# ychalier/transflow

Hardware: AMD Instinct MI355X
Metric: frames/sec (Farneback+remap) (higher is better)
Workload: dtype f32; 1 GPU; 4k: one clip of T=256 3840x2160 uint8 frames sharded over the ranks (rank r owns pairs shard_range(255, r, 1) + a one-frame halo), Farneback pyr_scale=0.5 levels=5 winsize=15 iterations=3 poly_n=5 poly_sigma=1.2 flags=0, BACKWARD post_process, moveref layer (reset random p=0.5 through a float mask, u drawn on the GPU), 1 RGB pixmap source, render; clip_frames=256, equal_batches=False

## Files before the change

transflow_amd/csrc/common.h:

```cpp
#pragma once
#include <hip/hip_runtime.h>

#include <cstdarg>
#include <cstdint>
#include <cstdio>
#include <cstdlib>
#include <string>
#include <vector>

#include "../../include/tfhip.h"

#define TF_API extern "C" __attribute__((visibility("default")))

namespace tf {

int set_error(int code, const char *fmt, ...) __attribute__((format(printf, 2, 3)));
hipStream_t stream();
hipStream_t main_stream();
int side_stream(int which, hipStream_t *out);
int ensure_init();

enum Opt { OPT_FB_FUSED = 0, OPT_FB_FUSE_MIN_PX, OPT_FB_NO_SHARE, OPT_FB_NO_OVERLAP, OPT_REMAP_PX, OPT_REMAP_NO_PACK, OPT_REMAP_KEEP_RGBA,
           OPT_PROF_LEVELS, OPT_FB_EXACT_SUMS, OPT_FB_CHAIN, OPT_FB_SEGS, OPT_REMAP_QUAD, OPT_JD_PAR_SUB_BYTES,
           OPT_JD_PAR_GROUP_SUBS, OPT_JD_PAR_STAGED, OPT_REMAP_LEAN, OPT_COUNT };
long option(Opt which);

#ifdef TF_EXPERIMENT
inline long tune(const char *env, long dflt)
{
    const char *v = getenv(env);
    return v ? atol(v) : dflt;
}
inline const char *tune_str(const char *env) { return getenv(env); }
#else
constexpr long tune(const char *, long dflt) { return dflt; }
constexpr const char *tune_str(const char *) { return nullptr; }
#endif

struct StreamScope {
    explicit StreamScope(hipStream_t s);
    ~StreamScope();
    hipStream_t prev;
};

#define TF_HIP(expr)                                                                              \
    do {                                                                                          \
        hipError_t _e = (expr);                                                                   \
        if (_e != hipSuccess)                                                                     \
            return tf::set_error(TF_ERR_HIP, "%s failed: %s (%s:%d)", #expr, hipGetErrorString(_e), \
                                 __FILE__, __LINE__);                                             \
    } while (0)

#define TF_TRY(expr)        \
    do {                    \
        int _rc = (expr);   \
        if (_rc != TF_OK)   \
            return _rc;     \
    } while (0)

#define TF_REQUIRE(cond, ...)                         \
    do {                                              \
        if (!(cond))                                  \
            return tf::set_error(TF_ERR_ARG, __VA_ARGS__); \
    } while (0)

struct ProfScope {
    explicit ProfScope(const char *name);
    ~ProfScope();
    const char *name;
    hipEvent_t a, b;
};
bool prof_enabled();

template <typename K, typename... Args>
inline int launch(const char *name, K kernel, dim3 grid, dim3 block, size_t smem, Args... args)
{
    if (grid.x == 0 || grid.y == 0 || grid.z == 0)
        return TF_OK;
    {
        ProfScope ps(name);
        hipLaunchKernelGGL(kernel, grid, block, smem, stream(), args...);
    }
    hipError_t e = hipGetLastError();
    if (e != hipSuccess)
        return set_error(TF_ERR_HIP, "launch %s failed: %s", name, hipGetErrorString(e));
    return TF_OK;
}

struct DevBuf {
    void *p = nullptr;
    size_t bytes = 0;
    bool borrowed = false;
    DevBuf() = default;
    DevBuf(const DevBuf &) = delete;
    DevBuf &operator=(const DevBuf &) = delete;
    ~DevBuf() { release(); }
    int alloc(size_t n);
    void borrow(void *ptr, size_t n);
    void release();
    template <typename T> T *as() const { return reinterpret_cast<T *>(p); }
};

struct PinnedBuf {
    void *p = nullptr;
    PinnedBuf() = default;
    PinnedBuf(const PinnedBuf &) = delete;
    PinnedBuf &operator=(const PinnedBuf &) = delete;
    ~PinnedBuf() { release(); }
    int alloc(size_t n);
    void release();
    template <typename T> T *as() const { return reinterpret_cast<T *>(p); }
};

struct Event {
    hipEvent_t e = nullptr;
    Event() = default;
    Event(const Event &) = delete;
    Event &operator=(const Event &) = delete;
    ~Event() { release(); }
    int create();
    void release();
    operator hipEvent_t() const { return e; }
};

inline unsigned cdiv(size_t a, size_t b) { return (unsigned)((a + b - 1) / b); }

struct FastDiv {
    uint32_t m;
    int s1, s2;
};
inline FastDiv fast_div_setup(uint32_t d)
{
    int s = 0;
    while ((1ull << s) < d)
        s++;
    FastDiv f;
    f.m = (uint32_t)(((1ull << 32) * ((1ull << s) - d)) / d + 1);
    f.s1 = s < 1 ? s : 1;
    f.s2 = s > 1 ? s - 1 : 0;
    return f;
}
__device__ __forceinline__ uint32_t fast_div(uint32_t t, FastDiv f)
{
    const uint32_t hi = __umulhi(t, f.m);
    return (((t - hi) >> f.s1) + hi) >> f.s2;
}

__device__ __forceinline__ float clip_nan(float v, float lo, float hi) { return v != v ? v : fminf(fmaxf(v, lo), hi); }

__device__ __forceinline__ int clampi(int v, int lo, int hi) { return v < lo ? lo : (v > hi ? hi : v); }

struct PpLabels {
    const char *clip, *fwd_scatter, *fwd_resolve, *ops;
};
constexpr PpLabels PP_FB{"pp_clip", "pp_fwd_scatter", "pp_fwd_resolve", "pp_ops"};
constexpr PpLabels PP_FLOW{"flow_pp_clip", "flow_pp_fwd_scatter", "flow_pp_fwd_resolve", "flow_pp_ops"};
int pp_ops(float2 *flow, int W, int H, int n_ops, const tf_flow_op *ops, const float *mask_dev, const PpLabels &lb);
int pp_scatter(const float2 *flow, int W, int H, int *winner, const PpLabels &lb);
int pp_direction(void *flow, bool wide, int W, int H, int direction, int *winner, const PpLabels &lb);

}
```

transflow_amd/csrc/fb_pyramid.hip:

```cpp
#include "fb_common.h"

namespace {

#ifndef TF_PX_TH
#define TF_PX_TH 16
#endif
constexpr int PX_TW = 64, PX_TH = TF_PX_TH;

__global__ void k_polyexp(const float *__restrict__ img, float *__restrict__ R, int Wk, int Hk, PolyConst pc)
{
    extern __shared__ float s_mem[];
    const int n = pc.n;
    const int LW = PX_TW + 2 * n;
    const int LH = PX_TH + 2 * n;
    float *sI = s_mem;
    float *sT = s_mem + LH * LW;
    const int pi = blockIdx.z;
    const size_t Nk = (size_t)Wk * Hk;
    const float *src = img + (size_t)pi * Nk;
    const int x0 = blockIdx.x * PX_TW, y0 = blockIdx.y * PX_TH;
    for (int idx = threadIdx.x; idx < LH * LW; idx += blockDim.x) {
        int ry = idx / LW, cx = idx % LW;
        int y = clampi(y0 - n + ry, 0, Hk - 1), x = clampi(x0 - n + cx, 0, Wk - 1);
        sI[idx] = src[(size_t)y * Wk + x];
    }
    __syncthreads();
    for (int idx = threadIdx.x; idx < PX_TH * LW; idx += blockDim.x) {
        int ty = idx / LW, cx = idx % LW;
        int y = y0 + ty;
        const float c = sI[(ty + n) * LW + cx];
        float t0 = c * pc.g[0], t1 = 0.f, t2 = 0.f;
        for (int k = 1; k <= n; k++) {
            int ya = max(y - k, 0), yb = min(y + k, Hk - 1);
            float a = sI[(ya - y0 + n) * LW + cx];
            float b = sI[(yb - y0 + n) * LW + cx];
            float p = a + b;
            t0 = t0 + pc.g[k] * p;
            t1 = t1 + pc.xg[k] * (b - a);
            t2 = t2 + pc.xxg[k] * p;
        }
        if (y >= Hk) {
            t0 = t1 = t2 = 0.f;
        }
        sT[(0 * PX_TH + ty) * LW + cx] = t0;
        sT[(1 * PX_TH + ty) * LW + cx] = t1;
        sT[(2 * PX_TH + ty) * LW + cx] = t2;
    }
    __syncthreads();
    float *dst = R + (size_t)pi * 5 * Nk;
    for (int idx = threadIdx.x; idx < PX_TH * PX_TW; idx += blockDim.x) {
        int ty = idx / PX_TW, cx = idx % PX_TW;
        int x = x0 + cx, y = y0 + ty;
        if (x >= Wk || y >= Hk)
            continue;
        const float *T0 = sT + (0 * PX_TH + ty) * LW + cx + n;
        const float *T1 = sT + (1 * PX_TH + ty) * LW + cx + n;
        const float *T2 = sT + (2 * PX_TH + ty) * LW + cx + n;
        float g0 = pc.g[0];
        double b1 = T0[0] * g0, b2 = 0, b3 = T1[0] * g0, b4 = 0, b5 = T2[0] * g0, b6 = 0;
        for (int k = 1; k <= n; k++) {
            double tg = T0[k] + T0[-k];
            g0 = pc.g[k];
            b1 = __builtin_fma(tg, (double)g0, b1);
            b4 = __builtin_fma(tg, (double)pc.xxg[k], b4);
            b2 += (T0[k] - T0[-k]) * pc.xg[k];
            b3 += (T1[k] + T1[-k]) * g0;
            b6 += (T1[k] - T1[-k]) * pc.xg[k];
            b5 += (T2[k] + T2[-k]) * g0;
        }
        size_t o = (size_t)y * Wk + x;
        const float v[5] = {(float)(b3 * pc.ig11), (float)(b2 * pc.ig11), (float)(b1 * pc.ig03 + b5 * pc.ig33),
                            (float)(b1 * pc.ig03 + b4 * pc.ig33), (float)(b6 * pc.ig55)};
        r_store_px(dst, Nk, o, v);
    }
}

typedef float float2w __attribute__((ext_vector_type(2), aligned(4)));

template <int N>
__device__ __forceinline__ void polyexp_vertical4(const f32x2 (&v)[4 + 2 * N], const PolyConst &pc, float *T0, float *T1,
                                                  float *T2, int LW)
{
#pragma unroll
    for (int q = 0; q < 4; q++) {
        const f32x2 c = v[q + N];
        f32x2 t0 = c * pc.g[0], t1 = {0.f, 0.f}, t2 = {0.f, 0.f};
#pragma unroll
        for (int k = 1; k <= N; k++) {
            const f32x2 a = v[q + N - k], b = v[q + N + k];
            const f32x2 p = a + b;
            t0 = t0 + pc.g[k] * p;
            t1 = t1 + pc.xg[k] * (b - a);
            t2 = t2 + pc.xxg[k] * p;
        }
        *reinterpret_cast<f32x2 *>(T0 + q * LW) = t0;
        *reinterpret_cast<f32x2 *>(T1 + q * LW) = t1;
        *reinterpret_cast<f32x2 *>(T2 + q * LW) = t2;
    }
}

template <int N>
__global__ void __launch_bounds__(256)
k_polyexp_t(const float *__restrict__ img, float *__restrict__ R, int Wk, int Hk, PolyConst pc)
{
    constexpr int TW = PX_TW, TH = PX_TH, LW = TW + 2 * N, LH = TH + 2 * N;
    __shared__ float sI[LH * LW];
    __shared__ float sT[3][TH][LW];
    const int pi = blockIdx.z;
    const size_t Nk = (size_t)Wk * Hk;
    const float *src = img + (size_t)pi * Nk;
    const int x0 = blockIdx.x * TW, y0 = blockIdx.y * TH;
    for (int idx = threadIdx.x; idx < LH * LW; idx += 256) {
        int ry = idx / LW, cx = idx - ry * LW;
        int y = clampi(y0 - N + ry, 0, Hk - 1), x = clampi(x0 - N + cx, 0, Wk - 1);
        sI[idx] = src[(size_t)y * Wk + x];
    }
    __syncthreads();
    static_assert(LW % 2 == 0, "column pairs");
    for (int idx = threadIdx.x; idx < (TH / 4) * (LW / 2); idx += 256) {
        const int g = idx / (LW / 2), cx = 2 * (idx - g * (LW / 2));
        f32x2 v[4 + 2 * N];
#pragma unroll
        for (int j = 0; j < 4 + 2 * N; j++)
            v[j] = *reinterpret_cast<const f32x2 *>(&sI[(4 * g + j) * LW + cx]);
        polyexp_vertical4<N>(v, pc, &sT[0][4 * g][cx], &sT[1][4 * g][cx], &sT[2][4 * g][cx], LW);
    }
    __syncthreads();
    float *dst = R + (size_t)pi * 5 * Nk;
    for (int idx = threadIdx.x; idx < TH * (TW / 2); idx += 256) {
        const int ty = idx / (TW / 2), cp = idx - ty * (TW / 2);
        const int x = x0 + 2 * cp, y = y0 + ty;
        if (x >= Wk || y >= Hk)
            continue;
        float w0[2 + 2 * N], w1[2 + 2 * N], w2[2 + 2 * N];
#pragma unroll
        for (int j = 0; j < 2 + 2 * N; j++) {
            w0[j] = sT[0][ty][2 * cp + j];
            w1[j] = sT[1][ty][2 * cp + j];
            w2[j] = sT[2][ty][2 * cp + j];
        }
        float out[2][5];
#pragma unroll
        for (int q = 0; q < 2; q++) {
            const float *T0 = w0 + q + N, *T1 = w1 + q + N, *T2 = w2 + q + N;
            float g0 = pc.g[0];
            double b1 = T0[0] * g0, b2 = 0, b3 = T1[0] * g0, b4 = 0, b5 = T2[0] * g0, b6 = 0;
#pragma unroll
            for (int k = 1; k <= N; k++) {
                double tg = T0[k] + T0[-k];
                g0 = pc.g[k];
                b1 = __builtin_fma(tg, (double)g0, b1);
                b4 = __builtin_fma(tg, (double)pc.xxg[k], b4);
                b2 += (T0[k] - T0[-k]) * pc.xg[k];
                b3 += (T1[k] + T1[-k]) * g0;
                b6 += (T1[k] - T1[-k]) * pc.xg[k];
                b5 += (T2[k] + T2[-k]) * g0;
            }
            out[q][0] = (float)(b3 * pc.ig11);
            out[q][1] = (float)(b2 * pc.ig11);
            out[q][2] = (float)(b1 * pc.ig03 + b5 * pc.ig33);
            out[q][3] = (float)(b1 * pc.ig03 + b4 * pc.ig33);
            out[q][4] = (float)(b6 * pc.ig55);
        }
        const size_t o = (size_t)y * Wk + x;
        if (x + 1 < Wk)
            r_store_px2(dst, Nk, o, out[0], out[1]);
        else
            r_store_px(dst, Nk, o, out[0]);
    }
}

template <int N, int TW, int TH>
__device__ __forceinline__ void tile_expansion(const float *sI, float (*sT)[TH][TW + 2 * N], int x0, int y0, int xr0,
                                               int yr0, int W, int H, const PolyConst &pc, float *dst, size_t Nk)
{
    constexpr int LW = TW + 2 * N;
    const bool interior = x0 - N >= 0 && x0 + TW - 1 + N <= W - 1 && y0 - N >= 0 && y0 + TH - 1 + N <= H - 1;
    for (int idx = threadIdx.x; idx < (TH / 4) * (LW / 2); idx += 256) {
        const int g = idx / (LW / 2), cx = 2 * (idx - g * (LW / 2));
        f32x2 v[4 + 2 * N];
        if (interior) {
#pragma unroll
            for (int j = 0; j < 4 + 2 * N; j++)
                v[j] = *reinterpret_cast<const f32x2 *>(&sI[(4 * g + j) * LW + cx]);
        } else {
            const int xa = clampi(x0 - N + cx, 0, W - 1) - xr0, xb = clampi(x0 - N + cx + 1, 0, W - 1) - xr0;
#pragma unroll
            for (int j = 0; j < 4 + 2 * N; j++) {
                const float *row = sI + (clampi(y0 - N + 4 * g + j, 0, H - 1) - yr0) * LW;
                v[j] = f32x2{row[xa], row[xb]};
            }
        }
        polyexp_vertical4<N>(v, pc, &sT[0][4 * g][cx], &sT[1][4 * g][cx], &sT[2][4 * g][cx], LW);
    }
    __syncthreads();
    for (int idx = threadIdx.x; idx < TH * (TW / 2); idx += 256) {
        const int ty = idx / (TW / 2), cp = idx - ty * (TW / 2);
        const int x = x0 + 2 * cp, y = y0 + ty;
        if (x >= W || y >= H)
            continue;
        float w0[2 + 2 * N], w1[2 + 2 * N], w2[2 + 2 * N];
#pragma unroll
        for (int j = 0; j < 2 + 2 * N; j++) {
            w0[j] = sT[0][ty][2 * cp + j];
            w1[j] = sT[1][ty][2 * cp + j];
            w2[j] = sT[2][ty][2 * cp + j];
        }
        float out[2][5];
#pragma unroll
        for (int q = 0; q < 2; q++) {
            const float *T0 = w0 + q + N, *T1 = w1 + q + N, *T2 = w2 + q + N;
            float g0 = pc.g[0];
            double b1 = T0[0] * g0, b2 = 0, b3 = T1[0] * g0, b4 = 0, b5 = T2[0] * g0, b6 = 0;
#pragma unroll
            for (int k = 1; k <= N; k++) {
                double tg = T0[k] + T0[-k];
                g0 = pc.g[k];
                b1 = __builtin_fma(tg, (double)g0, b1);
                b4 = __builtin_fma(tg, (double)pc.xxg[k], b4);
                b2 += (T0[k] - T0[-k]) * pc.xg[k];
                b3 += (T1[k] + T1[-k]) * g0;
                b6 += (T1[k] - T1[-k]) * pc.xg[k];
                b5 += (T2[k] + T2[-k]) * g0;
            }
            out[q][0] = (float)(b3 * pc.ig11);
            out[q][1] = (float)(b2 * pc.ig11);
            out[q][2] = (float)(b1 * pc.ig03 + b5 * pc.ig33);
            out[q][3] = (float)(b1 * pc.ig03 + b4 * pc.ig33);
            out[q][4] = (float)(b6 * pc.ig55);
        }
        const size_t o = (size_t)y * W + x;
        if (x + 1 < W)
            r_store_px2(dst, Nk, o, out[0], out[1]);
        else
            r_store_px(dst, Nk, o, out[0]);
    }
}

#ifndef TF_EXP_TH0
#define TF_EXP_TH0 16
#endif
#ifndef TF_EXP_TH1
#define TF_EXP_TH1 24
#endif
template <int N>
__global__ void __launch_bounds__(256)
k_level0_polyexp_t(const uint8_t *__restrict__ frames, const int2 *__restrict__ pairs, float *__restrict__ R, int W,
                   int H, float kc, float k1, PolyConst pc)
{
    constexpr int TW = 64, TH = TF_EXP_TH0, LW = TW + 2 * N, LH = TH + 2 * N;
    constexpr int SW = ((LW + 2 + 3 + 3) + 3) & ~3, SH = LH + 2;
    constexpr int RS = (LW + 3) & ~3;
    static_assert(SW >= RS + 4 + 4 && (SH * SW) % 16 == 0, "a group's three dwords stay inside its staged row; sRow 16-byte aligned");
    constexpr int BYTES_A = SH * SW + SH * RS * 4, BYTES_T = 3 * TH * LW * 4;
    constexpr int BYTES_U = ((BYTES_A > BYTES_T ? BYTES_A : BYTES_T) + 15) & ~15;
    __shared__ __attribute__((aligned(16))) uint8_t s_u[BYTES_U];
    __shared__ float sI[LH * LW];
    uint8_t *sS = s_u;
    float *sRow = reinterpret_cast<float *>(s_u + SH * SW);
    float(*sT)[TH][LW] = reinterpret_cast<float(*)[TH][LW]>(s_u);
    const int pi = blockIdx.z;
    const int2 pr = pairs[pi >> 1];
    const uint8_t *src = frames + (size_t)((pi & 1) ? pr.y : pr.x) * W * H;
    const size_t Nk = (size_t)W * H;
    const int x0 = blockIdx.x * TW, y0 = blockIdx.y * TH;
    const int lane = threadIdx.x & 63, wave = threadIdx.x >> 6;
    const int xr0 = max(x0 - N, 0), xr1 = min(x0 + TW - 1 + N, W - 1);
    const int yr0 = max(y0 - N, 0), yr1 = min(y0 + TH - 1 + N, H - 1);
    const int ny = yr1 - yr0 + 1;
    const int xs = (xr0 - 1) & ~3, off = xr0 - 1 - xs;
    const int ncols = xr1 + 1 - xs + 1;
    const bool dwords = (W & 3) == 0 && xs >= 0 && xs + ((ncols + 3) & ~3) <= W;
    constexpr int U = 8;
    if (dwords) {
        const int nq = (ncols + 3) >> 2;
        for (int c = lane; c < nq; c += 64) {
            for (int j0 = wave; j0 < ny + 2; j0 += 4 * U) {
                uint32_t v[U];
#pragma unroll
                for (int u = 0; u < U; u++) {
                    int ry = j0 + 4 * u;
                    if (ry < ny + 2)
                        v[u] = *reinterpret_cast<const uint32_t *>(src + (size_t)reflect101_near(yr0 - 1 + ry, H) * W + xs + 4 * c);
                }
#pragma unroll
                for (int u = 0; u < U; u++) {
                    int ry = j0 + 4 * u;
                    if (ry < ny + 2)
                        *reinterpret_cast<uint32_t *>(sS + ry * SW + 4 * c) = v[u];
                }
            }
        }
    } else {
        for (int c = lane; c < ncols; c += 64) {
            const int x = reflect101_near(xs + c, W);
            for (int j0 = wave; j0 < ny + 2; j0 += 4 * U) {
                uint8_t v[U];
#pragma unroll
                for (int u = 0; u < U; u++) {
                    int ry = j0 + 4 * u;
                    if (ry < ny + 2)
                        v[u] = src[(size_t)reflect101_near(yr0 - 1 + ry, H) * W + x];
                }
#pragma unroll
                for (int u = 0; u < U; u++) {
                    int ry = j0 + 4 * u;
                    if (ry < ny + 2)
                        sS[ry * SW + c] = v[u];
                }
            }
        }
    }
    __syncthreads();
    for (int idx = threadIdx.x; idx < (ny + 2) * (RS / 4); idx += 256) {
        const int ry = idx / (RS / 4), cx = 4 * (idx - ry * (RS / 4));
        const uint32_t *q = reinterpret_cast<const uint32_t *>(sS + ry * SW + cx);
        const uint32_t d0 = q[0], d1 = q[1], d2 = q[2];
        const uint32_t lo = __builtin_amdgcn_alignbyte(d1, d0, off), hi = __builtin_amdgcn_alignbyte(d2, d1, off);
        const float b0 = (float)(lo & 0xff), b1 = (float)((lo >> 8) & 0xff), b2 = (float)((lo >> 16) & 0xff),
                    b3 = (float)(lo >> 24), b4 = (float)(hi & 0xff), b5 = (float)((hi >> 8) & 0xff);
        float *o = sRow + ry * RS + cx;
        *reinterpret_cast<f32x2 *>(o) = f32x2{b1 * kc + (b0 + b2) * k1, b2 * kc + (b1 + b3) * k1};
        *reinterpret_cast<f32x2 *>(o + 2) = f32x2{b3 * kc + (b2 + b4) * k1, b4 * kc + (b3 + b5) * k1};
    }
    __syncthreads();
    for (int idx = threadIdx.x; idx < ny * (RS / 4); idx += 256) {
        const int ry = idx / (RS / 4), cx = 4 * (idx - ry * (RS / 4));
        const float *c = sRow + (ry + 1) * RS + cx;
        const f32x4 m = *reinterpret_cast<const f32x4 *>(c), dn = *reinterpret_cast<const f32x4 *>(c + RS),
                    up = *reinterpret_cast<const f32x4 *>(c - RS);
        f32x4 v = kc * m;
        v += k1 * (dn + up);
        float *o = sI + ry * LW + cx;
        *reinterpret_cast<f32x2 *>(o) = f32x2{v.x, v.y};
        if (cx + 2 < LW)
            *reinterpret_cast<f32x2 *>(o + 2) = f32x2{v.z, v.w};
    }
    __syncthreads();
    tile_expansion<N, TW, TH>(sI, sT, x0, y0, xr0, yr0, W, H, pc, R + (size_t)pi * 5 * Nk, Nk);
}

template <int N>
__global__ void __launch_bounds__(256)
k_level1_polyexp_t(const uint8_t *__restrict__ frames, const int2 *__restrict__ pairs, float *__restrict__ R, int W,
                   int H, float kc, float k1, PolyConst pc)
{
    constexpr int TW = 64, TH = TF_EXP_TH1, LW = TW + 2 * N, LH = TH + 2 * N;
    constexpr int SW = ((2 * LW + 2 + 3 + 3) + 3) & ~3, SH = 2 * LH + 2;
    constexpr int BYTES_A = SH * SW, BYTES_T = 3 * TH * LW * 4;
    constexpr int BYTES_U = ((BYTES_A > BYTES_T ? BYTES_A : BYTES_T) + 15) & ~15;
    __shared__ __attribute__((aligned(16))) uint8_t s_u[BYTES_U];
    __shared__ float sI[LH * LW];
    uint8_t *sS = s_u;
    float(*sT)[TH][LW] = reinterpret_cast<float(*)[TH][LW]>(s_u);
    const int Wk = W >> 1, Hk = H >> 1;
    const int pi = blockIdx.z;
    const int2 pr = pairs[pi >> 1];
    const uint8_t *src = frames + (size_t)((pi & 1) ? pr.y : pr.x) * W * H;
    const size_t Nk = (size_t)Wk * Hk;
    const int x0 = blockIdx.x * TW, y0 = blockIdx.y * TH;
    const int lane = threadIdx.x & 63, wave = threadIdx.x >> 6;
    const int xr0 = max(x0 - N, 0), xr1 = min(x0 + TW - 1 + N, Wk - 1);
    const int yr0 = max(y0 - N, 0), yr1 = min(y0 + TH - 1 + N, Hk - 1);
    const int ny = yr1 - yr0 + 1;
    const int cfirst = 2 * xr0 - 1, rfirst = 2 * yr0 - 1, nrows = 2 * ny + 2;
    const int xs = cfirst >= 0 ? (cfirst & ~3) : cfirst, off = cfirst - xs;
    const int ncols = 2 * xr1 + 2 - xs + 1;
    const bool dwords = (W & 3) == 0 && xs >= 0 && (xs & 3) == 0 && xs + ((ncols + 3) & ~3) <= W;
    constexpr int U = 8;
    if (dwords) {
        const int nq = (ncols + 3) >> 2;
        for (int c = lane; c < nq; c += 64) {
            for (int j0 = wave; j0 < nrows; j0 += 4 * U) {
                uint32_t v[U];
#pragma unroll
                for (int u = 0; u < U; u++) {
                    int ry = j0 + 4 * u;
                    if (ry < nrows)
                        v[u] = *reinterpret_cast<const uint32_t *>(src + (size_t)reflect101_near(rfirst + ry, H) * W + xs + 4 * c);
                }
#pragma unroll
                for (int u = 0; u < U; u++) {
                    int ry = j0 + 4 * u;
                    if (ry < nrows)
                        *reinterpret_cast<uint32_t *>(sS + ry * SW + 4 * c) = v[u];
                }
            }
        }
    } else {
        for (int c = lane; c < ncols; c += 64) {
            const int x = reflect101_near(xs + c, W);
            for (int j0 = wave; j0 < nrows; j0 += 4 * U) {
                uint8_t v[U];
#pragma unroll
                for (int u = 0; u < U; u++) {
                    int ry = j0 + 4 * u;
                    if (ry < nrows)
                        v[u] = src[(size_t)reflect101_near(rfirst + ry, H) * W + x];
                }
#pragma unroll
                for (int u = 0; u < U; u++) {
                    int ry = j0 + 4 * u;
                    if (ry < nrows)
                        sS[ry * SW + c] = v[u];
                }
            }
        }
    }
    __syncthreads();
    static_assert(LW % 2 == 0 && SW >= 2 * LW + 8, "2 x 2 blocks; a block's three dwords stay inside its staged row");
    for (int idx = threadIdx.x; idx < ((ny + 1) >> 1) * (LW / 2); idx += 256) {
        const int by2 = idx / (LW / 2), ry = 2 * by2, cx = 2 * (idx - by2 * (LW / 2));
        float rp[6][4];
#pragma unroll
        for (int dy = 0; dy < 6; dy++) {
            const uint32_t *q = reinterpret_cast<const uint32_t *>(sS + (2 * ry + dy) * SW + 2 * cx);
            const uint32_t d0 = q[0], d1 = q[1], d2 = q[2];
            const uint32_t lo = __builtin_amdgcn_alignbyte(d1, d0, off), hi = __builtin_amdgcn_alignbyte(d2, d1, off);
            const float b0 = (float)(lo & 0xff), b1 = (float)((lo >> 8) & 0xff), b2 = (float)((lo >> 16) & 0xff),
                        b3 = (float)(lo >> 24), b4 = (float)(hi & 0xff), b5 = (float)((hi >> 8) & 0xff);
            rp[dy][0] = b1 * kc + (b0 + b2) * k1;
            rp[dy][1] = b2 * kc + (b1 + b3) * k1;
            rp[dy][2] = b3 * kc + (b2 + b4) * k1;
            rp[dy][3] = b4 * kc + (b3 + b5) * k1;
        }
#pragma unroll
        for (int a = 0; a < 2; a++) {
            float out[2];
#pragma unroll
            for (int b = 0; b < 2; b++) {
                float v00 = kc * rp[2 * a + 1][2 * b], v01 = kc * rp[2 * a + 1][2 * b + 1];
                float v10 = kc * rp[2 * a + 2][2 * b], v11 = kc * rp[2 * a + 2][2 * b + 1];
                v00 += k1 * (rp[2 * a + 2][2 * b] + rp[2 * a][2 * b]);
                v01 += k1 * (rp[2 * a + 2][2 * b + 1] + rp[2 * a][2 * b + 1]);
                v10 += k1 * (rp[2 * a + 3][2 * b] + rp[2 * a + 1][2 * b]);
                v11 += k1 * (rp[2 * a + 3][2 * b + 1] + rp[2 * a + 1][2 * b + 1]);
                const float h0 = v00 * (1.f - 0.5f) + v01 * 0.5f, h1 = v10 * (1.f - 0.5f) + v11 * 0.5f;
                out[b] = h0 * (1.f - 0.5f) + h1 * 0.5f;
            }
            if (ry + a < ny)
                *reinterpret_cast<f32x2 *>(sI + (ry + a) * LW + cx) = f32x2{out[0], out[1]};
        }
    }
    __syncthreads();
    tile_expansion<N, TW, TH>(sI, sT, x0, y0, xr0, yr0, Wk, Hk, pc, R + (size_t)pi * 5 * Nk, Nk);
}

}

namespace tf {
namespace fb {

int fb_polyexp(tf_fb *fb, int w, int h, const ImageRun &run, int k)
{
    const int n = fb->pc.n;
    dim3 grid(cdiv(w, PX_TW), cdiv(h, PX_TH), run.n);
    if (n == 5)
        return launch(lvl_name("fb_polyexp", k), k_polyexp_t<5>, grid, dim3(256), 0, (const float *)fb->imgk(k),
                      fb->Rk(k, run), w, h, fb->pc);
    if (n == 7)
        return launch(lvl_name("fb_polyexp", k), k_polyexp_t<7>, grid, dim3(256), 0, (const float *)fb->imgk(k),
                      fb->Rk(k, run), w, h, fb->pc);
    size_t smem = ((size_t)(PX_TH + 2 * n) * (PX_TW + 2 * n) + 3 * (size_t)PX_TH * (PX_TW + 2 * n)) * sizeof(float);
    return launch(lvl_name("fb_polyexp_generic", k), k_polyexp, grid, dim3(256), smem,
                  (const float *)fb->imgk(k), fb->Rk(k, run), w, h, fb->pc);
}

static bool fb_can_fuse_level(tf_fb *fb, int k)
{
    static const bool off = tune("TF_FB_NO_A1A2", 0) != 0;
    const Level &L = *fb->lv[k];
    return !off && L.W == fb->W && L.H == fb->H && L.ksz == 3 && (fb->pc.n == 5 || fb->pc.n == 7);
}

static bool fb_can_fuse_half_level(tf_fb *fb, int k)
{
    static const bool off = tune("TF_FB_NO_A1A2", 0) != 0;
    const Level &L = *fb->lv[k];
    return !off && 2 * L.W == fb->W && 2 * L.H == fb->H && L.ksz == 3 && (fb->pc.n == 5 || fb->pc.n == 7);
}

static int fb_level1_polyexp(tf_fb *fb, int k, const ImageRun &run)
{
    Level &L = *fb->lv[k];
    dim3 grid(cdiv(L.W, 64), cdiv(L.H, TF_EXP_TH1), run.n);
    const float kc = L.kern_host[1], k1 = L.kern_host[2];
    if (fb->pc.n == 5)
        return launch(lvl_name("fb_level_polyexp", k), k_level1_polyexp_t<5>, grid, dim3(256), 0,
                      (const uint8_t *)fb->frames.as<uint8_t>(), fb->image_list(run), fb->Rk(k, run), fb->W,
                      fb->H, kc, k1, fb->pc);
    return launch(lvl_name("fb_level_polyexp", k), k_level1_polyexp_t<7>, grid, dim3(256), 0,
                  (const uint8_t *)fb->frames.as<uint8_t>(), fb->image_list(run), fb->Rk(k, run), fb->W, fb->H,
                  kc, k1, fb->pc);
}

static int fb_level0_polyexp(tf_fb *fb, int k, const ImageRun &run)
{
    Level &L = *fb->lv[k];
    dim3 grid(cdiv(L.W, 64), cdiv(L.H, TF_EXP_TH0), run.n);
    const float kc = L.kern_host[1], k1 = L.kern_host[2];
    if (fb->pc.n == 5)
        return launch(lvl_name("fb_level_polyexp", k), k_level0_polyexp_t<5>, grid, dim3(256), 0,
                      (const uint8_t *)fb->frames.as<uint8_t>(), fb->image_list(run), fb->Rk(k, run),
                      L.W, L.H, kc, k1, fb->pc);
    return launch(lvl_name("fb_level_polyexp", k), k_level0_polyexp_t<7>, grid, dim3(256), 0,
                  (const uint8_t *)fb->frames.as<uint8_t>(), fb->image_list(run), fb->Rk(k, run), L.W,
                  L.H, kc, k1, fb->pc);
}

int fb_expand_level(tf_fb *fb, int k, const ImageRun &run, bool standalone)
{
    if (fb_can_fuse_level(fb, k))
        return fb_level0_polyexp(fb, k, run);
    if (fb_can_fuse_half_level(fb, k))
        return fb_level1_polyexp(fb, k, run);
    TF_TRY(fb_level_image(fb, k, run, standalone));
    return fb_polyexp(fb, fb->lv[k]->W, fb->lv[k]->H, run, k);
}

}
}
```

transflow_amd/csrc/runtime.hip:

```cpp
#include <cstring>
#include <map>
#include <mutex>

#include "common.h"

#include <cstdlib>

namespace tf {

static thread_local std::string g_last_error;
static std::mutex g_mu;
static bool g_inited = false;
static int g_device = 0;
static hipStream_t g_stream = nullptr;

int set_error(int code, const char *fmt, ...)
{
    char buf[1024];
    va_list ap;
    va_start(ap, fmt);
    vsnprintf(buf, sizeof(buf), fmt, ap);
    va_end(ap);
    g_last_error = buf;
    return code;
}

struct OptDef {
    const char *name;
    long value, lo, hi;
};
static OptDef g_opts[OPT_COUNT] = {
    {"fb_fused", -1, -1, 1},
    {"fb_fuse_min_px", 4000000, 0, 1l << 40},
    {"fb_no_share", 0, 0, 1},
    {"fb_no_overlap", 0, 0, 1},
    {"remap_px", 4, 1, 4},
    {"remap_no_pack", 0, 0, 2},
    {"remap_keep_rgba", 0, 0, 1},
    {"prof_levels", 0, 0, 1},
    {"fb_exact_sums", 0, 0, 1},
    {"fb_chain", -1, -1, 1},
    {"fb_segs", 0, 0, 64},
    {"remap_quad", 1, 0, 1},
    {"jd_par_sub_bytes", 0, 0, 1024},
    {"jd_par_group_subs", 0, 0, 256},
    {"jd_par_staged", 0, 0, 1},
    {"remap_lean", 1, 0, 1},
};
long option(Opt which) { return g_opts[which].value; }

static thread_local hipStream_t g_override = nullptr;
static thread_local hipStream_t g_thread_main = nullptr;
static hipStream_t g_thread_streams[3] = {nullptr, nullptr, nullptr};

hipStream_t main_stream() { return g_thread_main ? g_thread_main : g_stream; }
hipStream_t stream() { return g_override ? g_override : main_stream(); }

static hipStream_t g_side[5] = {nullptr, nullptr, nullptr, nullptr, nullptr};
int side_stream(int which, hipStream_t *out)
{
    TF_REQUIRE(which >= 0 && which <= 4, "side_stream: bad index");
    TF_TRY(ensure_init());
    std::lock_guard<std::mutex> lk(g_mu);
    if (!g_side[which]) {
        int least = 0, greatest = 0;
        TF_HIP(hipDeviceGetStreamPriorityRange(&least, &greatest));
        TF_HIP(hipStreamCreateWithPriority(&g_side[which], hipStreamNonBlocking, (which == 0 || which >= 3) ? least : greatest));
    }
    *out = g_side[which];
    return TF_OK;
}

StreamScope::StreamScope(hipStream_t s) : prev(g_override) { g_override = s; }
StreamScope::~StreamScope() { g_override = prev; }

static int init_device(int device)
{
    std::lock_guard<std::mutex> lk(g_mu);
    if (g_inited) {
        if (device != g_device)
            return set_error(TF_ERR_STATE, "tf_init(%d): library already bound to device %d", device, g_device);
        TF_HIP(hipSetDevice(g_device));
        return TF_OK;
    }
    int n = 0;
    TF_HIP(hipGetDeviceCount(&n));
    if (device < 0 || device >= n)
        return set_error(TF_ERR_ARG, "tf_init: device %d out of range (%d visible)", device, n);
    TF_HIP(hipSetDevice(device));
    hipDeviceProp_t prop;
    TF_HIP(hipGetDeviceProperties(&prop, device));
    if (strncmp(prop.gcnArchName, "gfx950", 6) != 0)
        return set_error(TF_ERR_UNSUPPORTED, "tf_init: device %d is %s; this library is built for gfx950 only",
                         device, prop.gcnArchName);
    {
        int least = 0, greatest = 0;
        TF_HIP(hipDeviceGetStreamPriorityRange(&least, &greatest));
        TF_HIP(hipStreamCreateWithPriority(&g_stream, hipStreamNonBlocking, greatest));
    }
    g_device = device;
    g_inited = true;
    return TF_OK;
}

int ensure_init()
{
    if (g_inited)
        return hipSetDevice(g_device) == hipSuccess ? TF_OK : set_error(TF_ERR_HIP, "hipSetDevice failed");
    return init_device(0);
}

int DevBuf::alloc(size_t n)
{
    release();
    if (n == 0)
        return TF_OK;
    TF_HIP(hipMalloc(&p, n));
    bytes = n;
    return TF_OK;
}

void DevBuf::borrow(void *ptr, size_t n)
{
    release();
    p = ptr;
    bytes = n;
    borrowed = true;
}

void DevBuf::release()
{
    if (p && !borrowed)
        (void)hipFree(p);
    p = nullptr;
    bytes = 0;
    borrowed = false;
}

int PinnedBuf::alloc(size_t n)
{
    release();
    TF_HIP(hipHostMalloc(&p, n, hipHostMallocDefault));
    return TF_OK;
}

void PinnedBuf::release()
{
    if (p)
        (void)hipHostFree(p);
    p = nullptr;
}

int Event::create()
{
    release();
    TF_HIP(hipEventCreateWithFlags(&e, hipEventDisableTiming));
    return TF_OK;
}

void Event::release()
{
    if (e)
        (void)hipEventDestroy(e);
    e = nullptr;
}

struct ProfRec {
    const char *name;
    hipEvent_t a, b;
};
static bool g_prof = false;
static std::mutex g_prof_mu;
static std::string g_prof_filter;
static std::vector<ProfRec> g_recs;
static std::vector<hipEvent_t> g_free_events;
static std::map<std::string, std::pair<long, double>> g_acc;

bool prof_enabled() { return g_prof; }

static hipEvent_t get_event_locked()
{
    if (!g_free_events.empty()) {
        hipEvent_t e = g_free_events.back();
        g_free_events.pop_back();
        return e;
    }
    hipEvent_t e;
    (void)hipEventCreate(&e);
    return e;
}

static void prof_drain_locked()
{
    if (g_recs.empty())
        return;
    (void)hipDeviceSynchronize();
    for (auto &r : g_recs) {
        float ms = 0;
        (void)hipEventElapsedTime(&ms, r.a, r.b);
        auto &acc = g_acc[r.name];
// ... 321 lines not shown
```

Measured before the change: 2153 frames/s.

## Walk fused polyexp blocks down several sub-tiles, reusing blurred halo rows

```diff
diff --git a/transflow_amd/csrc/common.h b/transflow_amd/csrc/common.h
--- a/transflow_amd/csrc/common.h
+++ b/transflow_amd/csrc/common.h
@@ -22,7 +22,7 @@
 
 enum Opt { OPT_FB_FUSED = 0, OPT_FB_FUSE_MIN_PX, OPT_FB_NO_SHARE, OPT_FB_NO_OVERLAP, OPT_REMAP_PX, OPT_REMAP_NO_PACK, OPT_REMAP_KEEP_RGBA,
            OPT_PROF_LEVELS, OPT_FB_EXACT_SUMS, OPT_FB_CHAIN, OPT_FB_SEGS, OPT_REMAP_QUAD, OPT_JD_PAR_SUB_BYTES,
-           OPT_JD_PAR_GROUP_SUBS, OPT_JD_PAR_STAGED, OPT_REMAP_LEAN, OPT_COUNT };
+           OPT_JD_PAR_GROUP_SUBS, OPT_JD_PAR_STAGED, OPT_REMAP_LEAN, OPT_FB_EXP_WALK, OPT_COUNT };
 long option(Opt which);
 
 #ifdef TF_EXPERIMENT
diff --git a/transflow_amd/csrc/fb_pyramid.hip b/transflow_amd/csrc/fb_pyramid.hip
--- a/transflow_amd/csrc/fb_pyramid.hip
+++ b/transflow_amd/csrc/fb_pyramid.hip
@@ -172,11 +172,11 @@
 
 template <int N, int TW, int TH>
 __device__ __forceinline__ void tile_expansion(const float *sI, float (*sT)[TH][TW + 2 * N], int x0, int y0, int xr0,
-                                               int yr0, int W, int H, const PolyConst &pc, float *dst, size_t Nk)
+                                               int yr0, int W, int H, const PolyConst &pc, float *dst, size_t Nk, int tid)
 {
     constexpr int LW = TW + 2 * N;
     const bool interior = x0 - N >= 0 && x0 + TW - 1 + N <= W - 1 && y0 - N >= 0 && y0 + TH - 1 + N <= H - 1;
-    for (int idx = threadIdx.x; idx < (TH / 4) * (LW / 2); idx += 256) {
+    for (int idx = tid; idx < (TH / 4) * (LW / 2); idx += 256) {
         const int g = idx / (LW / 2), cx = 2 * (idx - g * (LW / 2));
         f32x2 v[4 + 2 * N];
         if (interior) {
@@ -194,7 +194,7 @@
         polyexp_vertical4<N>(v, pc, &sT[0][4 * g][cx], &sT[1][4 * g][cx], &sT[2][4 * g][cx], LW);
     }
     __syncthreads();
-    for (int idx = threadIdx.x; idx < TH * (TW / 2); idx += 256) {
+    for (int idx = tid; idx < TH * (TW / 2); idx += 256) {
         const int ty = idx / (TW / 2), cp = idx - ty * (TW / 2);
         const int x = x0 + 2 * cp, y = y0 + ty;
         if (x >= W || y >= H)
@@ -237,14 +237,58 @@
     }
 }
 
+template <int N, int S>
+__device__ __forceinline__ void walk_constants(int &tid, PolyConst &pc, float &kc, float &k1, int &W, int &H, int &x0)
+{
+    if (S > 1) {
+        asm volatile("" : "+v"(tid));
+#pragma unroll
+        for (int k = 0; k <= N; k++)
+            asm volatile("" : "+s"(pc.g[k]), "+s"(pc.xg[k]), "+s"(pc.xxg[k]));
+        asm volatile("" : "+s"(kc), "+s"(k1), "+s"(W), "+s"(H), "+s"(x0));
+    }
+}
+
+template <int S, typename T, int U>
+__device__ __forceinline__ void walk_define(T (&v)[U])
+{
+    if (S > 1) {
+#pragma unroll
+        for (int u = 0; u < U; u++)
+            v[u] = 0;
+    }
+}
+
+template <int N, int LW>
+__device__ __forceinline__ int keep_blurred_rows(float *sI, int first, int n, int tid)
+{
+    constexpr int C = (2 * N * (LW / 2) + 255) / 256;
+    n = max(n, 0);
+    f32x2 v[C] = {};
+#pragma unroll
+    for (int u = 0; u < C; u++) {
+        const int idx = tid + 256 * u;
+        if (idx < n * (LW / 2))
+            v[u] = *reinterpret_cast<const f32x2 *>(sI + first * LW + 2 * idx);
+    }
+    __syncthreads();
+#pragma unroll
+    for (int u = 0; u < C; u++) {
+        const int idx = tid + 256 * u;
+        if (idx < n * (LW / 2))
+            *reinterpret_cast<f32x2 *>(sI + 2 * idx) = v[u];
+    }
+    return n;
+}
+
 #ifndef TF_EXP_TH0
 #define TF_EXP_TH0 16
 #endif
 #ifndef TF_EXP_TH1
 #define TF_EXP_TH1 24
 #endif
-template <int N>
-__global__ void __launch_bounds__(256)
+template <int N, int S>
+__global__ void __launch_bounds__(256) __attribute__((amdgpu_waves_per_eu(N <= 5 ? 6 : 4)))
 k_level0_polyexp_t(const uint8_t *__restrict__ frames, const int2 *__restrict__ pairs, float *__restrict__ R, int W,
                    int H, float kc, float k1, PolyConst pc)
 {
@@ -252,6 +296,7 @@
     constexpr int SW = ((LW + 2 + 3 + 3) + 3) & ~3, SH = LH + 2;
     constexpr int RS = (LW + 3) & ~3;
     static_assert(SW >= RS + 4 + 4 && (SH * SW) % 16 == 0, "a group's three dwords stay inside its staged row; sRow 16-byte aligned");
+    static_assert(TH >= N, "a sub-tile below the first has its whole upper halo inside the level");
     constexpr int BYTES_A = SH * SW + SH * RS * 4, BYTES_T = 3 * TH * LW * 4;
     constexpr int BYTES_U = ((BYTES_A > BYTES_T ? BYTES_A : BYTES_T) + 15) & ~15;
     __shared__ __attribute__((aligned(16))) uint8_t s_u[BYTES_U];
@@ -261,86 +306,99 @@
     float(*sT)[TH][LW] = reinterpret_cast<float(*)[TH][LW]>(s_u);
     const int pi = blockIdx.z;
     const int2 pr = pairs[pi >> 1];
-    const uint8_t *src = frames + (size_t)((pi & 1) ? pr.y : pr.x) * W * H;
-    const size_t Nk = (size_t)W * H;
-    const int x0 = blockIdx.x * TW, y0 = blockIdx.y * TH;
-    const int lane = threadIdx.x & 63, wave = threadIdx.x >> 6;
-    const int xr0 = max(x0 - N, 0), xr1 = min(x0 + TW - 1 + N, W - 1);
-    const int yr0 = max(y0 - N, 0), yr1 = min(y0 + TH - 1 + N, H - 1);
-    const int ny = yr1 - yr0 + 1;
-    const int xs = (xr0 - 1) & ~3, off = xr0 - 1 - xs;
-    const int ncols = xr1 + 1 - xs + 1;
-    const bool dwords = (W & 3) == 0 && xs >= 0 && xs + ((ncols + 3) & ~3) <= W;
-    constexpr int U = 8;
-    if (dwords) {
-        const int nq = (ncols + 3) >> 2;
-        for (int c = lane; c < nq; c += 64) {
-            for (int j0 = wave; j0 < ny + 2; j0 += 4 * U) {
-                uint32_t v[U];
-#pragma unroll
-                for (int u = 0; u < U; u++) {
-                    int ry = j0 + 4 * u;
-                    if (ry < ny + 2)
-                        v[u] = *reinterpret_cast<const uint32_t *>(src + (size_t)reflect101_near(yr0 - 1 + ry, H) * W + xs + 4 * c);
+    int tid = threadIdx.x, x0 = blockIdx.x * TW;
+    int kept = 0;
+#pragma unroll 1
+    for (int sub = 0; sub < S; sub++) {
+        const int y0 = (blockIdx.y * S + sub) * TH;
+        if (S > 1 && y0 >= H)
+            break;
+        walk_constants<N, S>(tid, pc, kc, k1, W, H, x0);
+        const int lane = tid & 63, wave = tid >> 6;
+        const uint8_t *src = frames + (size_t)((pi & 1) ? pr.y : pr.x) * W * H;
+        const size_t Nk = (size_t)W * H;
+        const int xr0 = max(x0 - N, 0), xr1 = min(x0 + TW - 1 + N, W - 1);
+        const int xs = (xr0 - 1) & ~3, off = xr0 - 1 - xs;
+        const int ncols = xr1 + 1 - xs + 1;
+        const bool dwords = (W & 3) == 0 && xs >= 0 && xs + ((ncols + 3) & ~3) <= W;
+        const int yr0 = max(y0 - N, 0), yr1 = min(y0 + TH - 1 + N, H - 1);
+        const int ys0 = yr0 + kept, ny = yr1 - ys0 + 1;
+        constexpr int U = 8;
+        if (dwords) {
+            const int nq = (ncols + 3) >> 2;
+            for (int c = lane; c < nq; c += 64) {
+                for (int j0 = wave; j0 < ny + 2; j0 += 4 * U) {
+                    uint32_t v[U];
+                    walk_define<S>(v);
+#pragma unroll
+                    for (int u = 0; u < U; u++) {
+                        int ry = j0 + 4 * u;
+                        if (ry < ny + 2)
+                            v[u] = *reinterpret_cast<const uint32_t *>(src + (size_t)reflect101_near(ys0 - 1 + ry, H) * W + xs + 4 * c);
+                    }
+#pragma unroll
+                    for (int u = 0; u < U; u++) {
+                        int ry = j0 + 4 * u;
+                        if (ry < ny + 2)
+                            *reinterpret_cast<uint32_t *>(sS + ry * SW + 4 * c) = v[u];
+                    }
                 }
-#pragma unroll
-                for (int u = 0; u < U; u++) {
-                    int ry = j0 + 4 * u;
-                    if (ry < ny + 2)
-                        *reinterpret_cast<uint32_t *>(sS + ry * SW + 4 * c) = v[u];
+            }
+        } else {
+            for (int c = lane; c < ncols; c += 64) {
+                const int x = reflect101_near(xs + c, W);
+                for (int j0 = wave; j0 < ny + 2; j0 += 4 * U) {
+                    uint8_t v[U];
+                    walk_define<S>(v);
+#pragma unroll
+                    for (int u = 0; u < U; u++) {
+                        int ry = j0 + 4 * u;
+                        if (ry < ny + 2)
+                            v[u] = src[(size_t)reflect101_near(ys0 - 1 + ry, H) * W + x];
+                    }
+#pragma unroll
+                    for (int u = 0; u < U; u++) {
+                        int ry = j0 + 4 * u;
+                        if (ry < ny + 2)
+                            sS[ry * SW + c] = v[u];
+                    }
                 }
             }
         }
-    } else {
-        for (int c = lane; c < ncols; c += 64) {
-            const int x = reflect101_near(xs + c, W);
-            for (int j0 = wave; j0 < ny + 2; j0 += 4 * U) {
-                uint8_t v[U];
-#pragma unroll
-                for (int u = 0; u < U; u++) {
-                    int ry = j0 + 4 * u;
-                    if (ry < ny + 2)
-                        v[u] = src[(size_t)reflect101_near(yr0 - 1 + ry, H) * W + x];
-                }
-#pragma unroll
-                for (int u = 0; u < U; u++) {
-                    int ry = j0 + 4 * u;
-                    if (ry < ny + 2)
-                        sS[ry * SW + c] = v[u];
-                }
-            }
-        }
-    }
-    __syncthreads();
-    for (int idx = threadIdx.x; idx < (ny + 2) * (RS / 4); idx += 256) {
-        const int ry = idx / (RS / 4), cx = 4 * (idx - ry * (RS / 4));
-        const uint32_t *q = reinterpret_cast<const uint32_t *>(sS + ry * SW + cx);
-        const uint32_t d0 = q[0], d1 = q[1], d2 = q[2];
-        const uint32_t lo = __builtin_amdgcn_alignbyte(d1, d0, off), hi = __builtin_amdgcn_alignbyte(d2, d1, off);
-        const float b0 = (float)(lo & 0xff), b1 = (float)((lo >> 8) & 0xff), b2 = (float)((lo >> 16) & 0xff),
-                    b3 = (float)(lo >> 24), b4 = (float)(hi & 0xff), b5 = (float)((hi >> 8) & 0xff);
-        float *o = sRow + ry * RS + cx;
-        *reinterpret_cast<f32x2 *>(o) = f32x2{b1 * kc + (b0 + b2) * k1, b2 * kc + (b1 + b3) * k1};
-        *reinterpret_cast<f32x2 *>(o + 2) = f32x2{b3 * kc + (b2 + b4) * k1, b4 * kc + (b3 + b5) * k1};
-    }
-    __syncthreads();
-    for (int idx = threadIdx.x; idx < ny * (RS / 4); idx += 256) {
-        const int ry = idx / (RS / 4), cx = 4 * (idx - ry * (RS / 4));
-        const float *c = sRow + (ry + 1) * RS + cx;
-        const f32x4 m = *reinterpret_cast<const f32x4 *>(c), dn = *reinterpret_cast<const f32x4 *>(c + RS),
-                    up = *reinterpret_cast<const f32x4 *>(c - RS);
-        f32x4 v = kc * m;
-        v += k1 * (dn + up);
-        float *o = sI + ry * LW + cx;
-        *reinterpret_cast<f32x2 *>(o) = f32x2{v.x, v.y};
-        if (cx + 2 < LW)
-            *reinterpret_cast<f32x2 *>(o + 2) = f32x2{v.z, v.w};
-    }
-    __syncthreads();
-    tile_expansion<N, TW, TH>(sI, sT, x0, y0, xr0, yr0, W, H, pc, R + (size_t)pi * 5 * Nk, Nk);
-}
-
-template <int N>
+        __syncthreads();
+        for (int idx = tid; idx < (ny + 2) * (RS / 4); idx += 256) {
+            const int ry = idx / (RS / 4), cx = 4 * (idx - ry * (RS / 4));
+            const uint32_t *q = reinterpret_cast<const uint32_t *>(sS + ry * SW + cx);
+            const uint32_t d0 = q[0], d1 = q[1], d2 = q[2];
+            const uint32_t lo = __builtin_amdgcn_alignbyte(d1, d0, off), hi = __builtin_amdgcn_alignbyte(d2, d1, off);
+            const float b0 = (float)(lo & 0xff), b1 = (float)((lo >> 8) & 0xff), b2 = (float)((lo >> 16) & 0xff),
+                        b3 = (float)(lo >> 24), b4 = (float)(hi & 0xff), b5 = (float)((hi >> 8) & 0xff);
+            float *o = sRow + ry * RS + cx;
+            *reinterpret_cast<f32x2 *>(o) = f32x2{b1 * kc + (b0 + b2) * k1, b2 * kc + (b1 + b3) * k1};
+            *reinterpret_cast<f32x2 *>(o + 2) = f32x2{b3 * kc + (b2 + b4) * k1, b4 * kc + (b3 + b5) * k1};
+        }
+        __syncthreads();
+        float *sNew = sI + kept * LW;
+        for (int idx = tid; idx < ny * (RS / 4); idx += 256) {
+            const int ry = idx / (RS / 4), cx = 4 * (idx - ry * (RS / 4));
+            const float *c = sRow + (ry + 1) * RS + cx;
+            const f32x4 m = *reinterpret_cast<const f32x4 *>(c), dn = *reinterpret_cast<const f32x4 *>(c + RS),
+                        up = *reinterpret_cast<const f32x4 *>(c - RS);
+            f32x4 v = kc * m;
+            v += k1 * (dn + up);
+            float *o = sNew + ry * LW + cx;
+            *reinterpret_cast<f32x2 *>(o) = f32x2{v.x, v.y};
+            if (cx + 2 < LW)
+                *reinterpret_cast<f32x2 *>(o + 2) = f32x2{v.z, v.w};
+        }
+        __syncthreads();
+        tile_expansion<N, TW, TH>(sI, sT, x0, y0, xr0, yr0, W, H, pc, R + (size_t)pi * 5 * Nk, Nk, tid);
+        if (S > 1 && sub + 1 < S)
+            kept = keep_blurred_rows<N, LW>(sI, y0 + TH - N - yr0, yr1 - (y0 + TH - N) + 1, tid);
+    }
+}
+
+template <int N, int S>
 __global__ void __launch_bounds__(256)
 k_level1_polyexp_t(const uint8_t *__restrict__ frames, const int2 *__restrict__ pairs, float *__restrict__ R, int W,
                    int H, float kc, float k1, PolyConst pc)
@@ -349,101 +407,116 @@
     constexpr int SW = ((2 * LW + 2 + 3 + 3) + 3) & ~3, SH = 2 * LH + 2;
     constexpr int BYTES_A = SH * SW, BYTES_T = 3 * TH * LW * 4;
     constexpr int BYTES_U = ((BYTES_A > BYTES_T ? BYTES_A : BYTES_T) + 15) & ~15;
+    static_assert(TH >= N, "a sub-tile below the first has its whole upper halo inside the level");
     __shared__ __attribute__((aligned(16))) uint8_t s_u[BYTES_U];
     __shared__ float sI[LH * LW];
     uint8_t *sS = s_u;
     float(*sT)[TH][LW] = reinterpret_cast<float(*)[TH][LW]>(s_u);
-    const int Wk = W >> 1, Hk = H >> 1;
     const int pi = blockIdx.z;
     const int2 pr = pairs[pi >> 1];
-    const uint8_t *src = frames + (size_t)((pi & 1) ? pr.y : pr.x) * W * H;
-    const size_t Nk = (size_t)Wk * Hk;
-    const int x0 = blockIdx.x * TW, y0 = blockIdx.y * TH;
-    const int lane = threadIdx.x & 63, wave = threadIdx.x >> 6;
-    const int xr0 = max(x0 - N, 0), xr1 = min(x0 + TW - 1 + N, Wk - 1);
-    const int yr0 = max(y0 - N, 0), yr1 = min(y0 + TH - 1 + N, Hk - 1);
-    const int ny = yr1 - yr0 + 1;
-    const int cfirst = 2 * xr0 - 1, rfirst = 2 * yr0 - 1, nrows = 2 * ny + 2;
-    const int xs = cfirst >= 0 ? (cfirst & ~3) : cfirst, off = cfirst - xs;
-    const int ncols = 2 * xr1 + 2 - xs + 1;
-    const bool dwords = (W & 3) == 0 && xs >= 0 && (xs & 3) == 0 && xs + ((ncols + 3) & ~3) <= W;
-    constexpr int U = 8;
-    if (dwords) {
-        const int nq = (ncols + 3) >> 2;
-        for (int c = lane; c < nq; c += 64) {
-            for (int j0 = wave; j0 < nrows; j0 += 4 * U) {
-                uint32_t v[U];
-#pragma unroll
-                for (int u = 0; u < U; u++) {
-                    int ry = j0 + 4 * u;
-                    if (ry < nrows)
-                        v[u] = *reinterpret_cast<const uint32_t *>(src + (size_t)reflect101_near(rfirst + ry, H) * W + xs + 4 * c);
+    int tid = threadIdx.x, x0 = blockIdx.x * TW;
+    int kept = 0;
+#pragma unroll 1
+    for (int sub = 0; sub < S; sub++) {
+        const int y0 = (blockIdx.y * S + sub) * TH;
+        if (S > 1 && y0 >= (H >> 1))
+            break;
+        walk_constants<N, S>(tid, pc, kc, k1, W, H, x0);
+        const int lane = tid & 63, wave = tid >> 6;
+        const int Wk = W >> 1, Hk = H >> 1;
+        const uint8_t *src = frames + (size_t)((pi & 1) ? pr.y : pr.x) * W * H;
+        const size_t Nk = (size_t)Wk * Hk;
+        const int xr0 = max(x0 - N, 0), xr1 = min(x0 + TW - 1 + N, Wk - 1);
+        const int cfirst = 2 * xr0 - 1;
+        const int xs = cfirst >= 0 ? (cfirst & ~3) : cfirst, off = cfirst - xs;
+        const int ncols = 2 * xr1 + 2 - xs + 1;
+        const bool dwords = (W & 3) == 0 && xs >= 0 && (xs & 3) == 0 && xs + ((ncols + 3) & ~3) <= W;
+        const int yr0 = max(y0 - N, 0), yr1 = min(y0 + TH - 1 + N, Hk - 1);
+        const int ys0 = yr0 + kept, ny = yr1 - ys0 + 1;
+        const int rfirst = 2 * ys0 - 1, nrows = 2 * ny + 2;
+        constexpr int U = 8;
+        if (dwords) {
+            const int nq = (ncols + 3) >> 2;
+            for (int c = lane; c < nq; c += 64) {
+                for (int j0 = wave; j0 < nrows; j0 += 4 * U) {
+                    uint32_t v[U];
+                    walk_define<S>(v);
+#pragma unroll
+                    for (int u = 0; u < U; u++) {
+                        int ry = j0 + 4 * u;
+                        if (ry < nrows)
+                            v[u] = *reinterpret_cast<const uint32_t *>(src + (size_t)reflect101_near(rfirst + ry, H) * W + xs + 4 * c);
+                    }
+#pragma unroll
+                    for (int u = 0; u < U; u++) {
+                        int ry = j0 + 4 * u;
+                        if (ry < nrows)
+                            *reinterpret_cast<uint32_t *>(sS + ry * SW + 4 * c) = v[u];
+                    }
                 }
-#pragma unroll
-                for (int u = 0; u < U; u++) {
-                    int ry = j0 + 4 * u;
-                    if (ry < nrows)
-                        *reinterpret_cast<uint32_t *>(sS + ry * SW + 4 * c) = v[u];
+            }
+        } else {
+            for (int c = lane; c < ncols; c += 64) {
+                const int x = reflect101_near(xs + c, W);
+                for (int j0 = wave; j0 < nrows; j0 += 4 * U) {
+                    uint8_t v[U];
+                    walk_define<S>(v);
+#pragma unroll
+                    for (int u = 0; u < U; u++) {
+                        int ry = j0 + 4 * u;
+                        if (ry < nrows)
+                            v[u] = src[(size_t)reflect101_near(rfirst + ry, H) * W + x];
+                    }
+#pragma unroll
+                    for (int u = 0; u < U; u++) {
+                        int ry = j0 + 4 * u;
+                        if (ry < nrows)
+                            sS[ry * SW + c] = v[u];
+                    }
                 }
             }
         }
-    } else {
-        for (int c = lane; c < ncols; c += 64) {
-            const int x = reflect101_near(xs + c, W);
-            for (int j0 = wave; j0 < nrows; j0 += 4 * U) {
-                uint8_t v[U];
-#pragma unroll
-                for (int u = 0; u < U; u++) {
-                    int ry = j0 + 4 * u;
-                    if (ry < nrows)
-                        v[u] = src[(size_t)reflect101_near(rfirst + ry, H) * W + x];
+        __syncthreads();
+        static_assert(LW % 2 == 0 && SW >= 2 * LW + 8, "2 x 2 blocks; a block's three dwords stay inside its staged row");
+        float *sNew = sI + kept * LW;
+        for (int idx = tid; idx < ((ny + 1) >> 1) * (LW / 2); idx += 256) {
+            const int by2 = idx / (LW / 2), ry = 2 * by2, cx = 2 * (idx - by2 * (LW / 2));
+            float rp[6][4];
+#pragma unroll
+            for (int dy = 0; dy < 6; dy++) {
+                const uint32_t *q = reinterpret_cast<const uint32_t *>(sS + (2 * ry + dy) * SW + 2 * cx);
+                const uint32_t d0 = q[0], d1 = q[1], d2 = q[2];
+                const uint32_t lo = __builtin_amdgcn_alignbyte(d1, d0, off), hi = __builtin_amdgcn_alignbyte(d2, d1, off);
+                const float b0 = (float)(lo & 0xff), b1 = (float)((lo >> 8) & 0xff), b2 = (float)((lo >> 16) & 0xff),
+                            b3 = (float)(lo >> 24), b4 = (float)(hi & 0xff), b5 = (float)((hi >> 8) & 0xff);
+                rp[dy][0] = b1 * kc + (b0 + b2) * k1;
+                rp[dy][1] = b2 * kc + (b1 + b3) * k1;
+                rp[dy][2] = b3 * kc + (b2 + b4) * k1;
+                rp[dy][3] = b4 * kc + (b3 + b5) * k1;
+            }
+#pragma unroll
+            for (int a = 0; a < 2; a++) {
+                float out[2];
+#pragma unroll
+                for (int b = 0; b < 2; b++) {
+                    float v00 = kc * rp[2 * a + 1][2 * b], v01 = kc * rp[2 * a + 1][2 * b + 1];
+                    float v10 = kc * rp[2 * a + 2][2 * b], v11 = kc * rp[2 * a + 2][2 * b + 1];
+                    v00 += k1 * (rp[2 * a + 2][2 * b] + rp[2 * a][2 * b]);
+                    v01 += k1 * (rp[2 * a + 2][2 * b + 1] + rp[2 * a][2 * b + 1]);
+                    v10 += k1 * (rp[2 * a + 3][2 * b] + rp[2 * a + 1][2 * b]);
+                    v11 += k1 * (rp[2 * a + 3][2 * b + 1] + rp[2 * a + 1][2 * b + 1]);
+                    const float h0 = v00 * (1.f - 0.5f) + v01 * 0.5f, h1 = v10 * (1.f - 0.5f) + v11 * 0.5f;
+                    out[b] = h0 * (1.f - 0.5f) + h1 * 0.5f;
                 }
-#pragma unroll
-                for (int u = 0; u < U; u++) {
-                    int ry = j0 + 4 * u;
-                    if (ry < nrows)
-                        sS[ry * SW + c] = v[u];
-                }
-            }
-        }
-    }
-    __syncthreads();
-    static_assert(LW % 2 == 0 && SW >= 2 * LW + 8, "2 x 2 blocks; a block's three dwords stay inside its staged row");
-    for (int idx = threadIdx.x; idx < ((ny + 1) >> 1) * (LW / 2); idx += 256) {
-        const int by2 = idx / (LW / 2), ry = 2 * by2, cx = 2 * (idx - by2 * (LW / 2));
-        float rp[6][4];
-#pragma unroll
-        for (int dy = 0; dy < 6; dy++) {
-            const uint32_t *q = reinterpret_cast<const uint32_t *>(sS + (2 * ry + dy) * SW + 2 * cx);
-            const uint32_t d0 = q[0], d1 = q[1], d2 = q[2];
-            const uint32_t lo = __builtin_amdgcn_alignbyte(d1, d0, off), hi = __builtin_amdgcn_alignbyte(d2, d1, off);
-            const float b0 = (float)(lo & 0xff), b1 = (float)((lo >> 8) & 0xff), b2 = (float)((lo >> 16) & 0xff),
-                        b3 = (float)(lo >> 24), b4 = (float)(hi & 0xff), b5 = (float)((hi >> 8) & 0xff);
-            rp[dy][0] = b1 * kc + (b0 + b2) * k1;
-            rp[dy][1] = b2 * kc + (b1 + b3) * k1;
-            rp[dy][2] = b3 * kc + (b2 + b4) * k1;
-            rp[dy][3] = b4 * kc + (b3 + b5) * k1;
-        }
-#pragma unroll
-        for (int a = 0; a < 2; a++) {
-            float out[2];
-#pragma unroll
-            for (int b = 0; b < 2; b++) {
-                float v00 = kc * rp[2 * a + 1][2 * b], v01 = kc * rp[2 * a + 1][2 * b + 1];
-                float v10 = kc * rp[2 * a + 2][2 * b], v11 = kc * rp[2 * a + 2][2 * b + 1];
-                v00 += k1 * (rp[2 * a + 2][2 * b] + rp[2 * a][2 * b]);
-                v01 += k1 * (rp[2 * a + 2][2 * b + 1] + rp[2 * a][2 * b + 1]);
-                v10 += k1 * (rp[2 * a + 3][2 * b] + rp[2 * a + 1][2 * b]);
-                v11 += k1 * (rp[2 * a + 3][2 * b + 1] + rp[2 * a + 1][2 * b + 1]);
-                const float h0 = v00 * (1.f - 0.5f) + v01 * 0.5f, h1 = v10 * (1.f - 0.5f) + v11 * 0.5f;
-                out[b] = h0 * (1.f - 0.5f) + h1 * 0.5f;
-            }
-            if (ry + a < ny)
-                *reinterpret_cast<f32x2 *>(sI + (ry + a) * LW + cx) = f32x2{out[0], out[1]};
-        }
-    }
-    __syncthreads();
-    tile_expansion<N, TW, TH>(sI, sT, x0, y0, xr0, yr0, Wk, Hk, pc, R + (size_t)pi * 5 * Nk, Nk);
+                if (ry + a < ny)
+                    *reinterpret_cast<f32x2 *>(sNew + (ry + a) * LW + cx) = f32x2{out[0], out[1]};
+            }
+        }
+        __syncthreads();
+        tile_expansion<N, TW, TH>(sI, sT, x0, y0, xr0, yr0, Wk, Hk, pc, R + (size_t)pi * 5 * Nk, Nk, tid);
+        if (S > 1 && sub + 1 < S)
+            kept = keep_blurred_rows<N, LW>(sI, y0 + TH - N - yr0, yr1 - (y0 + TH - N) + 1, tid);
+    }
 }
 
 }
@@ -480,32 +553,55 @@
     return !off && 2 * L.W == fb->W && 2 * L.H == fb->H && L.ksz == 3 && (fb->pc.n == 5 || fb->pc.n == 7);
 }
 
+#ifndef TF_EXP_WALK0
+#define TF_EXP_WALK0 1
+#endif
+#ifndef TF_EXP_WALK1
+#define TF_EXP_WALK1 6
+#endif
+
+template <template <int, int> class K, int TH>
+static int launch_walk(tf_fb *fb, int k, const ImageRun &run, int best, int fw, int fh)
+{
+    Level &L = *fb->lv[k];
+    const long opt = option(OPT_FB_EXP_WALK);
+    const int n = fb->pc.n, S = opt > 0 ? (int)opt : n == 5 ? best : 1;
+    dim3 grid(cdiv(L.W, 64), cdiv(cdiv(L.H, TH), S), run.n);
+    const float kc = L.kern_host[1], k1 = L.kern_host[2];
+#define TF_WALK_CASE(S_)                                                                                              \
+    case S_:                                                                                                          \
+        return launch(lvl_name("fb_level_polyexp", k), n == 5 ? K<5, S_>::kernel : K<7, S_>::kernel, grid, dim3(256), \
+                      0, (const uint8_t *)fb->frames.as<uint8_t>(), fb->image_list(run), fb->Rk(k, run), fw, fh, kc,  \
+                      k1, fb->pc)
+    switch (S) {
+        TF_WALK_CASE(1);
+        TF_WALK_CASE(2);
+        TF_WALK_CASE(3);
+        TF_WALK_CASE(4);
+        TF_WALK_CASE(6);
+        TF_WALK_CASE(8);
+    }
+#undef TF_WALK_CASE
+    return set_error(TF_ERR_ARG, "fb_exp_walk: the fused expansion kernels are built for 1, 2, 3, 4, 6 and 8 sub-tiles, not %d", S);
+}
+
+template <int N, int S>
+struct Level0Walk {
+    static constexpr auto kernel = k_level0_polyexp_t<N, S>;
+};
+template <int N, int S>
+struct Level1Walk {
+    static constexpr auto kernel = k_level1_polyexp_t<N, S>;
+};
+
 static int fb_level1_polyexp(tf_fb *fb, int k, const ImageRun &run)
 {
-    Level &L = *fb->lv[k];
-    dim3 grid(cdiv(L.W, 64), cdiv(L.H, TF_EXP_TH1), run.n);
-    const float kc = L.kern_host[1], k1 = L.kern_host[2];
-    if (fb->pc.n == 5)
-        return launch(lvl_name("fb_level_polyexp", k), k_level1_polyexp_t<5>, grid, dim3(256), 0,
-                      (const uint8_t *)fb->frames.as<uint8_t>(), fb->image_list(run), fb->Rk(k, run), fb->W,
-                      fb->H, kc, k1, fb->pc);
-    return launch(lvl_name("fb_level_polyexp", k), k_level1_polyexp_t<7>, grid, dim3(256), 0,
-                  (const uint8_t *)fb->frames.as<uint8_t>(), fb->image_list(run), fb->Rk(k, run), fb->W, fb->H,
-                  kc, k1, fb->pc);
+    return launch_walk<Level1Walk, TF_EXP_TH1>(fb, k, run, TF_EXP_WALK1, fb->W, fb->H);
 }
 
 static int fb_level0_polyexp(tf_fb *fb, int k, const ImageRun &run)
 {
-    Level &L = *fb->lv[k];
-    dim3 grid(cdiv(L.W, 64), cdiv(L.H, TF_EXP_TH0), run.n);
-    const float kc = L.kern_host[1], k1 = L.kern_host[2];
-    if (fb->pc.n == 5)
-        return launch(lvl_name("fb_level_polyexp", k), k_level0_polyexp_t<5>, grid, dim3(256), 0,
-                      (const uint8_t *)fb->frames.as<uint8_t>(), fb->image_list(run), fb->Rk(k, run),
-                      L.W, L.H, kc, k1, fb->pc);
-    return launch(lvl_name("fb_level_polyexp", k), k_level0_polyexp_t<7>, grid, dim3(256), 0,
-                  (const uint8_t *)fb->frames.as<uint8_t>(), fb->image_list(run), fb->Rk(k, run), L.W,
-                  L.H, kc, k1, fb->pc);
+    return launch_walk<Level0Walk, TF_EXP_TH0>(fb, k, run, TF_EXP_WALK0, fb->lv[k]->W, fb->lv[k]->H);
 }
 
 int fb_expand_level(tf_fb *fb, int k, const ImageRun &run, bool standalone)
diff --git a/transflow_amd/csrc/runtime.hip b/transflow_amd/csrc/runtime.hip
--- a/transflow_amd/csrc/runtime.hip
+++ b/transflow_amd/csrc/runtime.hip
@@ -46,6 +46,7 @@
     {"jd_par_group_subs", 0, 0, 256},
     {"jd_par_staged", 0, 0, 1},
     {"remap_lean", 1, 0, 1},
+    {"fb_exp_walk", 0, 0, 8},
 };
 long option(Opt which) { return g_opts[which].value; }
 
```

Result: no change. 2156 frames/s (median of 5 runs) (+0.1%).
